# stdstu12/YUME

Measured on AMD Instinct MI355X. Metric: denoise-steps/sec (Yume-5B 720P, 33-frame latent), higher is better.
Workload: dtype bf16; 1 GPU; Yume-5B-720P random-init, 33-frame 704x1280 clip (latent 48x13x44x80, FramePack lfz=8, L=9460), ODE Euler steps of a 50-step shift-7 schedule, no CFG, one chain per GPU; num_layers=30, parallelism=dp1 (independent chains, replicated weights)

## Files before the change

include/yume_hip.h:

```cpp
#ifndef YUME_HIP_H
#define YUME_HIP_H

#include <stdint.h>

#ifdef __cplusplus
extern "C" {
#endif

#define YUME_OK 0
#define YUME_EINVAL (-1)
#define YUME_ELAUNCH (-2)
#define YUME_EUNSUP (-3)

const char* yume_last_error(void);
#define YUME_ABI_VERSION 9
int yume_abi_version(void);
const char* yume_target_arch(void);

int64_t yume_counter_workspace_bytes(void);
int yume_counter_workspace_init(void* ptr, int64_t bytes, void* stream);

int yume_calibrate_mfma(int64_t iters, int64_t workgroups, void* ticks, void* sink, void* stream);

int yume_adaln_modulate(const float* x, int64_t ldx, int64_t T, int64_t C, float eps,
                        const float* mul, const float* add, int64_t tab_stride,
                        const int32_t* row_idx, int add_one,
                        void* out, int64_t ldo, int out_kind, void* stream);

enum {
    YUME_EPI_BF16 = 0,
    YUME_EPI_BF16_GELU = 1,
    YUME_EPI_F32 = 2,
    YUME_EPI_RESID = 3,
    YUME_EPI_BF16_SPLITT = 4,
    YUME_EPI_BF16_GELU_ERF = 5,
    YUME_EPI_BF16_GEGLU = 6,
    YUME_EPI_MX_GELU = 7,
    YUME_EPI_MX6_GELU = 8
};
int yume_gemm_bf16(const void* A, int64_t lda, const void* W, int64_t ldw, const float* bias,
                   int64_t M, int64_t N, int64_t K, int epi,
                   void* out, int64_t ldo,
                   const float* gate, int64_t gate_stride, const int32_t* row_idx,
                   void* outT, int64_t ldt, int64_t n_split,
                   int variant, void* stream);

int64_t yume_gemm_workspace_bytes(void);
int yume_gemm_bf16_ws(const void* A, int64_t lda, const void* W, int64_t ldw, const float* bias,
                      int64_t M, int64_t N, int64_t K, int epi,
                      void* out, int64_t ldo,
                      const float* gate, int64_t gate_stride, const int32_t* row_idx,
                      void* outT, int64_t ldt, int64_t n_split,
                      int variant, void* workspace, int64_t workspace_bytes, void* stream);

int yume_quant_rows_e4m3(const void* x, int64_t ldx, int64_t R, int64_t K, void* q, int64_t ldq, float* scale, void* stream);
int yume_gemm_f8(const void* Aq, int64_t lda, const float* sa, const void* Wq, int64_t ldw, const float* sw,
                 const float* bias, int64_t M, int64_t N, int64_t K, int epi, void* out, int64_t ldo,
                 const float* gate, int64_t gate_stride, const int32_t* row_idx, void* stream);
int yume_gemm_f8_splitt(const void* Aq, int64_t lda, const float* sa, const void* Wq, int64_t ldw, const float* sw,
                        const float* bias, int64_t M, int64_t N, int64_t K,
                        void* out, int64_t ldo, void* outT, int64_t ldt, int64_t n_split, void* stream);

int yume_adaln_modulate_e4m3(const float* x, int64_t ldx, int64_t T, int64_t C, float eps, const float* mul,
                             const float* add, int64_t tab_stride, const int32_t* row_idx, int add_one,
                             void* q, int64_t ldq, float* scale, void* stream);
int yume_gemm_f8_mxout(const void* Aq, int64_t lda, const float* sa, const void* Wq, int64_t ldw, const float* sw,
                       const float* bias, int64_t M, int64_t N, int64_t K, int epi, void* out, int64_t ldo,
                       void* eo, int64_t ldeo, void* stream);
int yume_gemm_f8_mx(const void* Aq, int64_t lda, const void* ea, int64_t ldea, const void* Wq, int64_t ldw, const float* sw,
                    const float* bias, int64_t M, int64_t N, int64_t K, int epi, void* out, int64_t ldo,
                    const float* gate, int64_t gate_stride, const int32_t* row_idx, void* stream);

int yume_adaln_modulate_mx_e2m3(const float* x, int64_t ldx, int64_t T, int64_t C, float eps, const float* mul,
                                const float* add, int64_t tab_stride, const int32_t* row_idx, int add_one,
                                void* q, int64_t ldq, void* e, int64_t lde, void* stream);
int yume_gemm_f6_mx(const void* A6, int64_t lda, const void* ea, int64_t ldea, const void* W6, int64_t ldw, const void* ew, int64_t ldew,
                    const float* bias, int64_t M, int64_t N, int64_t K, int epi, void* out, int64_t ldo,
                    const float* gate, int64_t gate_stride, const int32_t* row_idx, void* stream);
int yume_gemm_f6_mxout(const void* A6, int64_t lda, const void* ea, int64_t ldea, const void* W6, int64_t ldw, const void* ew, int64_t ldew,
                       const float* bias, int64_t M, int64_t N, int64_t K, int epi, void* out, int64_t ldo,
                       void* eo, int64_t ldeo, void* stream);

int yume_quant_rows_i8(const void* x, int64_t ldx, int64_t R, int64_t K, void* q, int64_t ldq, float* scale, void* stream);
int yume_adaln_modulate_i8(const float* x, int64_t ldx, int64_t T, int64_t C, float eps, const float* mul,
                           const float* add, int64_t tab_stride, const int32_t* row_idx, int add_one,
                           void* q, int64_t ldq, float* scale, void* stream);
int yume_gemm_i8(const void* Aq, int64_t lda, const float* sa, const void* Wq, int64_t ldw, const float* sw,
                 const float* bias, int64_t M, int64_t N, int64_t K, int epi, void* out, int64_t ldo, void* stream);
int yume_gemm_i8_splitt(const void* Aq, int64_t lda, const float* sa, const void* Wq, int64_t ldw, const float* sw,
                        const float* bias, int64_t M, int64_t N, int64_t K,
                        void* out, int64_t ldo, void* outT, int64_t ldt, int64_t n_split, void* stream);

int yume_rmsnorm_rope(void* buf, int64_t ld, int64_t T, int64_t C, int nparts,
                      const float* w, float eps, const float* rope, int64_t D, void* stream);
int yume_rmsnorm_rows_periodic(void* buf, int64_t ld, int64_t T, int64_t C, const float* w, int64_t wperiod, float eps,
                               void* stream);

#define YUME_ATTN_Q_PRESCALED 0x100
#define YUME_ATTN_KV_PADDED 0x200
int yume_attn_fwd(const void* Q, int64_t ldq, const void* K, int64_t ldk, const void* Vt, int64_t ldvt,
                  void* O, int64_t ldo, int64_t Lq, int64_t Lk, int64_t H, float scale,
                  int accumulate, int variant, void* stream);
int64_t yume_attn_workspace_bytes(int64_t Lq, int64_t Lk, int64_t H);
int yume_attn_fwd_ws(const void* Q, int64_t ldq, const void* K, int64_t ldk, const void* Vt, int64_t ldvt,
                     void* O, int64_t ldo, int64_t Lq, int64_t Lk, int64_t H, float scale,
                     int accumulate, int variant, void* workspace, int64_t workspace_bytes, void* stream);
int yume_attn_fwd_kw(const void* Q, int64_t ldq, const void* K, int64_t ldk, const void* Vt, int64_t ldvt,
                     void* O, int64_t ldo, int64_t Lq, int64_t Lk, int64_t H, float scale,
                     int accumulate, int variant, void* workspace, int64_t workspace_bytes, float last_key_weight, void* stream);
int yume_attn_fwd_band(const void* Q, int64_t ldq, const void* K, int64_t ldk, const void* Vt, int64_t ldvt,
                       void* O, int64_t ldo, int64_t Lq, int64_t Lk, int64_t H, float scale, int accumulate, int variant,
                       int64_t q_pos0, int64_t win_left, int64_t win_right,
                       void* workspace, int64_t workspace_bytes, void* stream);
int yume_attn_fwd_seg(const void* Q, int64_t ldq, const void* const* K, int64_t ldk, const void* const* Vt, int64_t ldvt,
                      void* O, int64_t ldo, int64_t nseg, int64_t Lq_seg, int64_t seg_pitch, const int64_t* Lk, int64_t H,
                      float scale, int accumulate, int variant, const float* last_key_weight, void* stream);
int64_t yume_attn_batch_workspace_bytes(int64_t nseg, int64_t Lq_seg, int64_t Lk_seg, int64_t H);
int yume_attn_fwd_batch(const void* Q, int64_t ldq, const void* K, int64_t ldk, const void* Vt, int64_t ldvt,
                        void* O, int64_t ldo, int64_t nseg, int64_t Lq_seg, int64_t q_pitch,
                        int64_t Lk_seg, int64_t k_pitch, int64_t H, float scale, int accumulate, int variant,
                        void* workspace, int64_t workspace_bytes, void* stream);

int yume_quant_rows_mx_e4m3(const void* x, int64_t ldx, int64_t R, int64_t K, void* q, int64_t ldq, void* e, int64_t lde, void* stream);
int yume_attn_vt_mx_e4m3(const void* Vt, int64_t ldvt, int64_t C, int64_t Lk, void* Vt8, int64_t ldvt8, void* Ev, int64_t ldev, void* stream);
int yume_attn_fwd_f8mx(const void* Q8, int64_t ldq, const void* Eq, int64_t ldeq, const void* K8, int64_t ldk, const void* Ek, int64_t ldek,
                       const void* Vt8, int64_t ldvt8, const void* Ev, int64_t ldev, void* O, int64_t ldo,
                       int64_t Lq, int64_t Lk, int64_t H, void* stream);

int yume_linear_smallm_f32(const float* in, int64_t R, int64_t K, const void* W, int w_bf16,
                           const float* bias, int64_t N, int in_act, int out_act,
                           const float* add_table, float* out, void* stream);

int yume_sinusoidal_embed(const double* t, const int32_t* t_index, int64_t R, int64_t dim,
                          float* out, void* stream);

int yume_modulation_table(const float* tab, const float* e0, int64_t B, int64_t R, int64_t W,
// ... 69 lines not shown
```

yume_amd/_lib.py:

```python
import ctypes
import os
from ctypes import c_void_p, c_int, c_int64, c_float, c_char_p

_HERE = os.path.dirname(os.path.abspath(__file__))
LIB_PATH = os.environ.get("YUME_HIP_LIB") or os.path.join(_HERE, "lib", "libyume_hip.so")

_P, _I, _L, _F = c_void_p, c_int, c_int64, c_float

SIGNATURES = {
    "yume_last_error": [],
    "yume_abi_version": [],
    "yume_target_arch": [],
    "yume_counter_workspace_bytes": [],
    "yume_counter_workspace_init": [_P, _L, _P],
    "yume_calibrate_mfma": [_L, _L, _P, _P, _P],
    "yume_adaln_modulate": [_P, _L, _L, _L, _F, _P, _P, _L, _P, _I, _P, _L, _I, _P],
    "yume_adaln_modulate_e4m3": [_P, _L, _L, _L, _F, _P, _P, _L, _P, _I, _P, _L, _P, _P],
    "yume_gemm_bf16": [_P, _L, _P, _L, _P, _L, _L, _L, _I, _P, _L, _P, _L, _P, _P, _L, _L, _I, _P],
    "yume_gemm_workspace_bytes": [],
    "yume_gemm_bf16_ws": [_P, _L, _P, _L, _P, _L, _L, _L, _I, _P, _L, _P, _L, _P, _P, _L, _L, _I, _P, _L, _P],
    "yume_quant_rows_e4m3": [_P, _L, _L, _L, _P, _L, _P, _P],
    "yume_gemm_f8": [_P, _L, _P, _P, _L, _P, _P, _L, _L, _L, _I, _P, _L, _P, _L, _P, _P],
    "yume_gemm_f8_splitt": [_P, _L, _P, _P, _L, _P, _P, _L, _L, _L, _P, _L, _P, _L, _L, _P],
    "yume_gemm_f8_mxout": [_P, _L, _P, _P, _L, _P, _P, _L, _L, _L, _I, _P, _L, _P, _L, _P],
    "yume_gemm_f8_mx": [_P, _L, _P, _L, _P, _L, _P, _P, _L, _L, _L, _I, _P, _L, _P, _L, _P, _P],
    "yume_adaln_modulate_mx_e2m3": [_P, _L, _L, _L, _F, _P, _P, _L, _P, _I, _P, _L, _P, _L, _P],
    "yume_gemm_f6_mx": [_P, _L, _P, _L, _P, _L, _P, _L, _P, _L, _L, _L, _I, _P, _L, _P, _L, _P, _P],
    "yume_gemm_f6_mxout": [_P, _L, _P, _L, _P, _L, _P, _L, _P, _L, _L, _L, _I, _P, _L, _P, _L, _P],
    "yume_quant_rows_i8": [_P, _L, _L, _L, _P, _L, _P, _P],
    "yume_adaln_modulate_i8": [_P, _L, _L, _L, _F, _P, _P, _L, _P, _I, _P, _L, _P, _P],
    "yume_gemm_i8": [_P, _L, _P, _P, _L, _P, _P, _L, _L, _L, _I, _P, _L, _P],
    "yume_gemm_i8_splitt": [_P, _L, _P, _P, _L, _P, _P, _L, _L, _L, _P, _L, _P, _L, _L, _P],
    "yume_rmsnorm_f32": [_P, _L, _L, _L, _F, _P, _P, _L, _P],
    "yume_gemm_bf16_batched": [_P, _L, _L, _P, _L, _L, _L, _L, _L, _I, _P, _L, _L, _L, _I, _P],
    "yume_gemm_splitk_workspace_bytes": [_L, _L, _I],
    "yume_gemm_bf16_splitk": [_P, _L, _P, _L, _P, _L, _L, _L, _I, _P, _L, _I, _P, _P],
    "yume_softmax_bias_rows": [_P, _L, _L, _L, _L, _P, _L, _P, _L, _L, _P],
    "yume_rmsnorm_rows_periodic": [_P, _L, _L, _L, _P, _L, _F, _P],
    "yume_rmsnorm_rope": [_P, _L, _L, _L, _I, _P, _F, _P, _L, _P],
    "yume_attn_fwd": [_P, _L, _P, _L, _P, _L, _P, _L, _L, _L, _L, _F, _I, _I, _P],
    "yume_attn_workspace_bytes": [_L, _L, _L],
    "yume_attn_fwd_ws": [_P, _L, _P, _L, _P, _L, _P, _L, _L, _L, _L, _F, _I, _I, _P, _L, _P],
    "yume_attn_fwd_kw": [_P, _L, _P, _L, _P, _L, _P, _L, _L, _L, _L, _F, _I, _I, _P, _L, _F, _P],
    "yume_attn_fwd_band": [_P, _L, _P, _L, _P, _L, _P, _L, _L, _L, _L, _F, _I, _I, _L, _L, _L, _P, _L, _P],
    "yume_attn_fwd_seg": [_P, _L, _P, _L, _P, _L, _P, _L, _L, _L, _L, _P, _L, _F, _I, _I, _P, _P],
    "yume_attn_batch_workspace_bytes": [_L, _L, _L, _L],
    "yume_attn_fwd_batch": [_P, _L, _P, _L, _P, _L, _P, _L, _L, _L, _L, _L, _L, _L, _F, _I, _I, _P, _L, _P],
    "yume_quant_rows_mx_e4m3": [_P, _L, _L, _L, _P, _L, _P, _L, _P],
    "yume_attn_vt_mx_e4m3": [_P, _L, _L, _L, _P, _L, _P, _L, _P],
    "yume_attn_fwd_f8mx": [_P, _L, _P, _L, _P, _L, _P, _L, _P, _L, _P, _L, _P, _L, _L, _L, _L, _P],
    "yume_linear_smallm_f32": [_P, _L, _L, _P, _I, _P, _L, _I, _I, _P, _P, _P],
    "yume_sinusoidal_embed": [_P, _P, _L, _L, _P, _P],
    "yume_modulation_table": [_P, _P, _L, _L, _L, _P, _P],
    "yume_patch_gather": [_P, _I, _L, _L, _L, _L, _L, _L, _L, _L, _P, _L, _P],
    "yume_unpatchify": [_P, _L, _L, _L, _L, _L, _L, _L, _P, _P],
    "yume_cast_bf16": [_P, _L, _L, _L, _L, _P, _L, _P],
    "yume_transpose_bf16": [_P, _I, _L, _L, _L, _P, _L, _P],
    "yume_conv3d_cl": [_P, _P, _L, _L, _L, _L, _L, _P, _L, _P, _L, _I, _I, _I, _I, _I, _I, _I, _I, _I, _I, _L, _L, _L, _I, _P, _L,
                       _P, _L, _P, _P],
    "yume_vae_rmsnorm_silu": [_P, _L, _L, _L, _P, _P, _I, _P, _L, _P],
    "yume_vae_rmsnorm_silu_mx": [_P, _L, _L, _L, _P, _P, _I, _P, _L, _P, _L, _P],
    "yume_conv3d_cl_f8mx": [_P, _P, _P, _P, _L, _L, _L, _L, _L, _L, _P, _L, _P, _P, _L, _I, _I, _I, _I, _I, _I, _I, _I, _I, _I, _L, _L, _L,
                            _I, _P, _L, _P, _L, _P, _P],
    "yume_conv_up2_fold": [_P, _L, _L, _L, _L, _L, _P, _L, _P, _L, _P, _L, _P],
    "yume_vae_dupup_add": [_P, _L, _L, _L, _L, _L, _P, _L, _L, _L, _I, _I, _I, _P],
    "yume_vae_avgdown_add": [_P, _L, _L, _L, _L, _L, _P, _L, _L, _I, _I, _P],
    "yume_softmax_rows": [_P, _L, _L, _L, _F, _P, _L, _P],
    "yume_vae_pack_input": [_P, _I, _L, _L, _L, _L, _I, _P, _P, _P, _L, _P],
    "yume_frames_u8": [_P, _L, _L, _L, _L, _P, _P],
    "yume_frames_u8_trunc": [_P, _L, _L, _L, _L, _P, _P],
    "yume_vae_unpack_output": [_P, _L, _L, _L, _L, _L, _I, _P, _P, _F, _F, _P, _P],
}
_RES = {"yume_last_error": c_char_p, "yume_target_arch": c_char_p, "yume_gemm_splitk_workspace_bytes": c_int64, "yume_attn_workspace_bytes": c_int64,
        "yume_attn_batch_workspace_bytes": c_int64,
        "yume_counter_workspace_bytes": c_int64, "yume_gemm_workspace_bytes": c_int64}

_lib = None
ABI_VERSION = 9


def load():
    global _lib
    if _lib is not None:
        return _lib
    if not os.path.exists(LIB_PATH):
        raise RuntimeError(
            f"{LIB_PATH} is missing: the HIP extension has not been built. "
            "Run `python -c 'import __graft_entry__ as g; g.build()'` (or `python -m yume_amd.build`). "
            "There is no CPU/PyTorch fallback for the yume_amd hot path.")
    import torch
    lib = ctypes.CDLL(LIB_PATH)
    for name, argtypes in SIGNATURES.items():
        fn = getattr(lib, name)
        fn.argtypes = argtypes
        fn.restype = _RES.get(name, c_int)
    got, arch = int(lib.yume_abi_version()), lib.yume_target_arch()
    if got != ABI_VERSION or arch != b"gfx950":
        raise RuntimeError(f"{LIB_PATH} has ABI version {got} for {arch!r}, this binding needs {ABI_VERSION} for gfx950: "
                           "rebuild with `python -m yume_amd.build --force`")
    _lib = lib
    return lib


def check(rc, what):
    if rc != 0:
        msg = load().yume_last_error()
        raise RuntimeError(f"{what} failed (rc={rc}): {msg.decode() if msg else '?'}")
```

yume_amd/csrc/gemm_bf16.hip:

```cpp
#include "gemm_core.hpp"
#include "gemm_w4.hpp"

using namespace gemm_core;

namespace {
bool w4_auto() {
    static const bool on = [] { const char* v = getenv("YUME_GEMM_W4"); return !v || atoi(v) != 0; }();
    return on;
}
bool gemm_log() {
    static const bool on = [] { const char* v = getenv("YUME_GEMM_LOG"); return v && atoi(v) != 0; }();
    return on;
}
void gemm_log_line(const char* kernel, int64_t M, int64_t N, int64_t K, int epi, int variant, int64_t lda, int64_t ldw, int64_t ldo, int64_t ldt,
                   int64_t n_split, bool ws, int64_t batch) {
    fprintf(stderr, "[gemm_bf16] %s M=%lld N=%lld K=%lld epi=%d variant=%d lda=%lld ldw=%lld ldo=%lld ldt=%lld n_split=%lld ws=%d batch=%lld\n", kernel,
            (long long)M, (long long)N, (long long)K, epi, variant, (long long)lda, (long long)ldw, (long long)ldo, (long long)ldt, (long long)n_split,
            ws ? 1 : 0, (long long)batch);
}
}

extern "C" int64_t yume_gemm_workspace_bytes(void) { return gemm_w4::sk_workspace_bytes(gemm_w4::SK_MAX_SLOTS); }

extern "C" int yume_gemm_bf16(const void* A, int64_t lda, const void* W, int64_t ldw, const float* bias, int64_t M,
                              int64_t N, int64_t K, int epi, void* out, int64_t ldo, const float* gate,
                              int64_t gate_stride, const int32_t* row_idx, void* outT, int64_t ldt, int64_t n_split,
                              int variant, void* stream) {
    return yume_gemm_bf16_ws(A, lda, W, ldw, bias, M, N, K, epi, out, ldo, gate, gate_stride, row_idx, outT, ldt, n_split, variant, nullptr, 0, stream);
}

extern "C" int yume_gemm_bf16_ws(const void* A, int64_t lda, const void* W, int64_t ldw, const float* bias, int64_t M,
                                 int64_t N, int64_t K, int epi, void* out, int64_t ldo, const float* gate,
                                 int64_t gate_stride, const int32_t* row_idx, void* outT, int64_t ldt, int64_t n_split,
                                 int variant, void* workspace, int64_t workspace_bytes, void* stream) {
    YUME_REQUIRE(A && W && out, "gemm_bf16: NULL pointer");
    YUME_REQUIRE(M > 0 && N > 0 && K > 0, "gemm_bf16: empty problem M=%lld N=%lld K=%lld", (long long)M, (long long)N, (long long)K);
    YUME_REQUIRE(M < (1ll << 31) && N < (1ll << 31) && K < (1ll << 31), "gemm_bf16: dimension too large");
    YUME_REQUIRE((K % BK) == 0, "gemm_bf16: K=%lld must be a multiple of %d", (long long)K, BK);
    YUME_REQUIRE((N % 4) == 0, "gemm_bf16: N=%lld must be a multiple of 4", (long long)N);
    YUME_REQUIRE((lda % 8) == 0 && (ldw % 8) == 0, "gemm_bf16: lda/ldw must be multiples of 8 (16-byte rows)");
    YUME_REQUIRE((ldo % 4) == 0, "gemm_bf16: ldo must be a multiple of 4");
    YUME_REQUIRE(((uintptr_t)A % 16) == 0 && ((uintptr_t)W % 16) == 0 && ((uintptr_t)out % 16) == 0, "gemm_bf16: pointers must be 16-byte aligned");
    Problem p;
    p.W = (const unsigned short*)W; p.ldw = ldw;
    p.M = (int)M; p.N = (int)N; p.K = (int)K;
    p.tiles_m = (int)((M + BM - 1) / BM);
    p.tiles_n = (int)((N + BN - 1) / BN);
    p.group_m = 8;
    p.bsW = 0; p.bsO = 0;
    bool sk = false;
    if (variant == 0 && workspace != nullptr && w4_auto() && epi != YUME_EPI_BF16_GEGLU &&
        use_256(p, 0, epi != YUME_EPI_BF16_SPLITT || (n_split % 256) == 0) && gemm_w4::w4_applies(p, lda, epi) &&
        (epi != YUME_EPI_BF16_SPLITT || (ldt % 8) == 0)) {
        Problem q = p;
        q.tiles_m = (int)((M + 255) / 256);
        q.tiles_n = (int)((N + 255) / 256);
        gemm_w4::w4_sk_plan(q, workspace, workspace_bytes);
        sk = q.sk_wgs != 0;
    }
    if (!sk && variant == 0 && epi != YUME_EPI_BF16_GEGLU && use_256(p, 0, epi != YUME_EPI_BF16_SPLITT || (n_split % 256) == 0)) {
        const int64_t tn = (N + 255) / 256, tm = (M + 255) / 256, T = tm * tn, R = T % 256, full = T - R;
        const int64_t m_main = full / tn, M_main = m_main * 256, rem = M - M_main;
        if (R > 0 && R <= 96 && full >= 256 && m_main >= 1 && rem > 0 && rem <= 1024) {
            const int64_t osz = (epi == YUME_EPI_F32 || epi == YUME_EPI_RESID) ? 4 : 2;
            auto remainder = [&](void* s2) {
                return yume_gemm_bf16(reinterpret_cast<const unsigned short*>(A) + M_main * lda, lda, W, ldw, bias, rem, N, K, epi,
                                      reinterpret_cast<char*>(out) + M_main * ldo * osz, ldo, gate, gate_stride,
                                      row_idx ? row_idx + M_main : nullptr,
                                      outT ? reinterpret_cast<unsigned short*>(outT) + M_main : nullptr, ldt, n_split, 1, s2);
            };
            int rc = yume_gemm_bf16(A, lda, W, ldw, bias, M_main, N, K, epi, out, ldo, gate, gate_stride, row_idx, outT, ldt, n_split,
                                    w4_auto() ? 3 : 2, stream);
            if (rc != YUME_OK) return rc;
            return remainder(stream);
        }
    }
    PlainA al;
    al.A = (const unsigned short*)A; al.lda = lda; al.M = (int)M; al.bsA = 0;
    Epilogue e = {};
    e.bias = bias;
    e.out = out; e.ldo = ldo;
    e.gate = gate; e.gate_stride = gate_stride; e.row_idx = row_idx;
    e.outT = (unsigned short*)outT; e.ldt = ldt; e.n_split = (int)n_split;
    hipStream_t st = (hipStream_t)stream;
    const bool split_ok = epi != YUME_EPI_BF16_SPLITT || (n_split % 256) == 0;
    const bool big = use_256(p, variant == 3 ? 2 : variant, split_ok);
    const bool w4 = (variant == 3 || (variant == 0 && big && w4_auto())) && split_ok && gemm_w4::w4_applies(p, lda, epi) &&
                    (epi != YUME_EPI_BF16_SPLITT || (ldt % 8) == 0);
    if (gemm_log())
        gemm_log_line(epi == YUME_EPI_BF16_GEGLU ? "g256" : w4 ? (sk ? "w4+sk" : "w4") : big ? "g256" : "g128", M, N, K, epi, variant, lda, ldw, ldo, ldt,
                      n_split, workspace != nullptr, 1);
#define YUME_GO(E) (w4 ? gemm_w4::launch_w4(E, p, al, e, st, "gemm_bf16", variant == 0 ? workspace : nullptr, workspace_bytes) : big ? launch256<E>(p, al, e, st, "gemm_bf16") : launch<E>(p, al, e, st, "gemm_bf16"))
    switch (epi) {
        case YUME_EPI_BF16: return YUME_GO(YUME_EPI_BF16);
        case YUME_EPI_BF16_GELU: return YUME_GO(YUME_EPI_BF16_GELU);
        case YUME_EPI_BF16_GELU_ERF: return YUME_GO(YUME_EPI_BF16_GELU_ERF);
        case YUME_EPI_F32: return YUME_GO(YUME_EPI_F32);
        case YUME_EPI_RESID:
            YUME_REQUIRE(gate == nullptr || (gate_stride % 4) == 0, "gemm_bf16: gate_stride must be a multiple of 4");
            return YUME_GO(YUME_EPI_RESID);
        case YUME_EPI_BF16_GEGLU:
            YUME_REQUIRE((N % 8) == 0 && bias == nullptr, "gemm_bf16: GEGLU needs N %% 8 == 0 and no bias");
            return launch256<YUME_EPI_BF16_GEGLU>(p, al, e, st, "gemm_bf16");
        case YUME_EPI_BF16_SPLITT:
            YUME_REQUIRE(outT != nullptr && n_split >= 0 && (n_split % BN) == 0 && ldt >= M && (ldt % 4) == 0,
                         "gemm_bf16: SPLITT needs outT, n_split %% 128 == 0, ldt >= M and ldt %% 4 == 0");
            YUME_REQUIRE(((uintptr_t)outT % 16) == 0, "gemm_bf16: outT must be 16-byte aligned");
            return YUME_GO(YUME_EPI_BF16_SPLITT);
        default:
            yume_set_error("gemm_bf16: unknown epilogue %d", epi);
            return YUME_EINVAL;
    }
}

extern "C" int yume_gemm_bf16_batched(const void* A, int64_t lda, int64_t strideA, const void* W, int64_t ldw, int64_t strideW,
                                      int64_t M, int64_t N, int64_t K, int epi, void* out, int64_t ldo, int64_t strideO,
                                      int64_t batch, int variant, void* stream) {
    (void)variant;
    YUME_REQUIRE(A && W && out, "gemm_bf16_batched: NULL pointer");
    YUME_REQUIRE(epi == YUME_EPI_BF16 || epi == YUME_EPI_F32, "gemm_bf16_batched: only the plain bf16 / fp32 epilogues");
    YUME_REQUIRE(batch >= 1 && batch <= 65535, "gemm_bf16_batched: batch %lld", (long long)batch);
    YUME_REQUIRE(M > 0 && N > 0 && K > 0 && M < (1ll << 31) && N < (1ll << 31) && K < (1ll << 31), "gemm_bf16_batched: bad problem size");
    YUME_REQUIRE((K % BK) == 0 && (N % 4) == 0, "gemm_bf16_batched: K must be a multiple of %d and N of 4", BK);
    YUME_REQUIRE((lda % 8) == 0 && (ldw % 8) == 0 && (ldo % 4) == 0, "gemm_bf16_batched: lda/ldw must be multiples of 8, ldo of 4");
    YUME_REQUIRE((strideA % 8) == 0 && (strideW % 8) == 0 && (strideO % 8) == 0, "gemm_bf16_batched: strides must keep 16-byte alignment");
    YUME_REQUIRE(((uintptr_t)A % 16) == 0 && ((uintptr_t)W % 16) == 0 && ((uintptr_t)out % 16) == 0, "gemm_bf16_batched: pointers must be 16-byte aligned");
    Problem p;
    p.W = (const unsigned short*)W; p.ldw = ldw;
    p.M = (int)M; p.N = (int)N; p.K = (int)K;
    p.tiles_m = (int)((M + BM - 1) / BM);
    p.tiles_n = (int)((N + BN - 1) / BN);
    p.group_m = 8;
    p.bsW = strideW;
    p.bsO = strideO * (epi == YUME_EPI_F32 ? 4 : 2);
    PlainA al;
    al.A = (const unsigned short*)A; al.lda = lda; al.M = (int)M; al.bsA = strideA;
    Epilogue e = {};
    e.out = out; e.ldo = ldo;
    hipStream_t st = (hipStream_t)stream;
    if (gemm_log()) gemm_log_line("batched", M, N, K, epi, variant, lda, ldw, ldo, 0, 0, false, batch);
    if (epi == YUME_EPI_F32) return launch<YUME_EPI_F32>(p, al, e, st, "gemm_bf16_batched", (int)batch);
    return launch<YUME_EPI_BF16>(p, al, e, st, "gemm_bf16_batched", (int)batch);
}

namespace {
template <int EPI>
__global__ __launch_bounds__(256) void splitk_reduce_kernel(const float* __restrict__ ws, int splits, int64_t MN, int N,
                                                            const float* __restrict__ bias, void* __restrict__ out, int64_t ldo) {
    const int64_t nq = MN >> 2;
    for (int64_t i = (int64_t)blockIdx.x * blockDim.x + threadIdx.x; i < nq; i += (int64_t)gridDim.x * blockDim.x) {
        f32x4 v = *reinterpret_cast<const f32x4*>(ws + 4 * i);
        for (int s = 1; s < splits; ++s) v += *reinterpret_cast<const f32x4*>(ws + s * MN + 4 * i);
        const int64_t m = (4 * i) / N;
        const int n = (int)((4 * i) - m * N);
        if (bias) v += *reinterpret_cast<const f32x4*>(bias + n);
        if (EPI == YUME_EPI_F32) {
            *reinterpret_cast<f32x4*>(reinterpret_cast<float*>(out) + m * ldo + n) = v;
        } else if (EPI == YUME_EPI_RESID) {
            float* xo = reinterpret_cast<float*>(out) + m * ldo + n;
            *reinterpret_cast<f32x4*>(xo) = *reinterpret_cast<const f32x4*>(xo) + v;
        } else if (EPI == YUME_EPI_BF16_GEGLU) {
            const unsigned o = pack_bf16x2(v[1] * gelu_tanh(v[0]), v[3] * gelu_tanh(v[2]));
            *reinterpret_cast<unsigned*>(reinterpret_cast<unsigned short*>(out) + m * ldo + (n >> 1)) = o;
        } else {
            if (EPI == YUME_EPI_BF16_GELU) {
#pragma unroll
                for (int q = 0; q < 4; ++q) v[q] = gelu_tanh(v[q]);
            }
            if (EPI == YUME_EPI_BF16_GELU_ERF) {
#pragma unroll
                for (int q = 0; q < 4; ++q) v[q] = 0.5f * v[q] * (1.0f + erff(v[q] * 0.7071067811865476f));
            }
            u32x2 o;
            o[0] = pack_bf16x2(v[0], v[1]);
            o[1] = pack_bf16x2(v[2], v[3]);
            *reinterpret_cast<u32x2*>(reinterpret_cast<unsigned short*>(out) + m * ldo + n) = o;
        }
    }
}
}

extern "C" int64_t yume_gemm_splitk_workspace_bytes(int64_t M, int64_t N, int splits) { return (int64_t)splits * M * N * 4; }

extern "C" int yume_gemm_bf16_splitk(const void* A, int64_t lda, const void* W, int64_t ldw, const float* bias, int64_t M, int64_t N,
                                     int64_t K, int epi, void* out, int64_t ldo, int splits, void* workspace, void* stream) {
    YUME_REQUIRE(A && W && out && workspace, "gemm_bf16_splitk: NULL pointer");
    YUME_REQUIRE(splits >= 1 && splits <= 64 && (K % (splits * BK)) == 0, "gemm_bf16_splitk: K=%lld must be a multiple of splits*%d (splits=%d)",
                 (long long)K, BK, splits);
    YUME_REQUIRE(M > 0 && N > 0 && (N % 8) == 0 && (ldo % 4) == 0, "gemm_bf16_splitk: N must be a multiple of 8, ldo of 4");
    YUME_REQUIRE(((uintptr_t)workspace % 16) == 0 && ((uintptr_t)out % 16) == 0, "gemm_bf16_splitk: pointers must be 16-byte aligned");
    YUME_REQUIRE((M * N) % 4 == 0, "gemm_bf16_splitk: M*N must be a multiple of 4");
    const int64_t Ks = K / splits;
    int rc = yume_gemm_bf16_batched(A, lda, Ks, W, ldw, Ks, M, N, Ks, YUME_EPI_F32, workspace, N, M * N, splits, 1, stream);
    if (rc != YUME_OK) return rc;
    const int64_t MN = M * N;
    const unsigned grid = (unsigned)((MN / 4 + 255) / 256 > 16384 ? 16384 : (MN / 4 + 255) / 256);
    hipStream_t st = (hipStream_t)stream;
// ... 20 lines not shown
```

yume_amd/csrc/gemm_w4.hpp:

```cpp
#pragma once
#include "gemm_core.hpp"
#include "trace.hpp"

namespace gemm_w4 {
using namespace gemm_core;

constexpr int NTHR_W4 = 256;
constexpr int OPER_BYTES = 256 * 128;
constexpr int BUF_BYTES = 2 * OPER_BYTES;
constexpr int LDS_W4 = 2 * BUF_BYTES;

#define W4_AG8(n) "a" #n "0", "a" #n "1", "a" #n "2", "a" #n "3", "a" #n "4", "a" #n "5", "a" #n "6", "a" #n "7", "a" #n "8", "a" #n "9"
#define W4_AGPRS "a0", "a1", "a2", "a3", "a4", "a5", "a6", "a7", "a8", "a9", W4_AG8(1), W4_AG8(2), W4_AG8(3), W4_AG8(4), W4_AG8(5), W4_AG8(6), \
    W4_AG8(7), W4_AG8(8), W4_AG8(9), W4_AG8(10), W4_AG8(11), W4_AG8(12), W4_AG8(13), W4_AG8(14), W4_AG8(15), W4_AG8(16), W4_AG8(17), W4_AG8(18), \
    W4_AG8(19), W4_AG8(20), W4_AG8(21), W4_AG8(22), W4_AG8(23), W4_AG8(24), "a250", "a251", "a252", "a253", "a254", "a255"

#define W4_MFMA2(T0, X0, Y0, T1, X1, Y1)                                                                                                         \
    asm volatile("v_mfma_f32_16x16x32_bf16 a[%c4:%c5], %0, %1, a[%c4:%c5]\n\tv_mfma_f32_16x16x32_bf16 a[%c6:%c7], %2, %3, a[%c6:%c7]"             \
                 ::"v"(X0), "v"(Y0), "v"(X1), "v"(Y1), "n"((T0) * 4), "n"((T0) * 4 + 3), "n"((T1) * 4), "n"((T1) * 4 + 3) : "memory", W4_AGPRS)
#define W4_MFMA2_DMA(T0, X0, Y0, T1, X1, Y1, voff, sbase, lbase, loff)                                                                            \
    asm volatile("s_add_u32 m0, %10, %11\n\tv_mfma_f32_16x16x32_bf16 a[%c4:%c5], %0, %1, a[%c4:%c5]\n\tglobal_load_lds_dwordx4 %8, %9\n\t"         \
                 "v_mfma_f32_16x16x32_bf16 a[%c6:%c7], %2, %3, a[%c6:%c7]"                                                                       \
                 ::"v"(X0), "v"(Y0), "v"(X1), "v"(Y1), "n"((T0) * 4), "n"((T0) * 4 + 3), "n"((T1) * 4), "n"((T1) * 4 + 3), "v"(voff), "s"(sbase),   \
                 "s"(lbase), "n"(loff) : "memory", "scc", W4_AGPRS)
// ... 550 lines not shown
            tails = true;
            const int ntail = (p.sk_s - 1) * R;
            pc0 = (w - R) * p.sk_q;
            pc1 = min(ntail, pc0 + p.sk_q);
            if (pc0 >= pc1) return;
        }
    }
    for (int pc = pc0; pc < pc1; ++pc) {
        int t = head_t, j = 0, k0 = 0, k1 = nk, slot = -1, nslice = 1;
        if (p.sk_wgs && (int)blockIdx.x >= ndp) {
            if (tails) {
                j = 1 + pc / R;
                t = pc - (j - 1) * R;
                k0 = p.sk_lh + (j - 1) * p.sk_lt;
                k1 = j == p.sk_s - 1 ? nk : k0 + p.sk_lt;
                slot = pc;
            } else {
                k1 = p.sk_lh;
                nslice = p.sk_s;
            }
        }
        int m0, n0;
        tile_origin(p, tile0 + t, m0, n0);
        if (epi == YUME_EPI_BF16_SPLITT && n0 >= e.n_split) {
            w4_mainloop<false>(p, al, smem, m0, n0, k0, k1 - k0);
            w4_finish_piece<false>(p, e, epi, smem, m0, n0, slot, t, nslice);
        } else {
            w4_mainloop<true>(p, al, smem, m0, n0, k0, k1 - k0);
            w4_finish_piece<true>(p, e, epi, smem, m0, n0, slot, t, nslice);
        }
        if (pc + 1 < pc1) __syncthreads();
    }
    TRACE_STAMP(2);
}

inline bool w4_applies(const Problem& p, int64_t lda, int epi) {
    if (p.K < 3 * BK) return false;
#ifdef W4_EXPERIMENT
    if (epi != YUME_EPI_BF16) return false;
#endif
    if (255ll * lda * 2 + 128 >= (1ll << 32) || 255ll * p.ldw * 2 + 128 >= (1ll << 32)) return false;
    return epi == YUME_EPI_BF16 || epi == YUME_EPI_BF16_GELU || epi == YUME_EPI_BF16_GELU_ERF || epi == YUME_EPI_F32 || epi == YUME_EPI_RESID ||
           epi == YUME_EPI_BF16_SPLITT;
}

inline void w4_sk_plan(Problem& p, void* ws, int64_t ws_bytes) {
    p.sk_dp = 0; p.sk_tiles = 0; p.sk_wgs = 0; p.sk_s = 1; p.sk_q = 1; p.sk_lh = 0; p.sk_lt = 0; p.sk_ws = nullptr;
    static const bool on = [] { const char* v = getenv("YUME_GEMM_SK"); return !v || atoi(v) != 0; }();
    static const int ncu = [] {
        int d = 0, n = 0;
        if (hipGetDevice(&d) != hipSuccess || hipDeviceGetAttribute(&n, hipDeviceAttributeMultiprocessorCount, d) != hipSuccess) n = 0;
        return n;
    }();
    if (!on || ws == nullptr || ncu < 64 || ncu > SK_MAX_SLOTS || (ncu & 7) != 0) return;
    if (ws_bytes < sk_workspace_bytes(SK_MAX_SLOTS) || ((uintptr_t)ws & 15) != 0) return;
    const int T = p.tiles_m * p.tiles_n, nk = p.K / BK;
    const int R = T % ncu;
    if (R == 0 || T < ncu) return;
    static const int min_nk = [] { const char* v = getenv("YUME_GEMM_SK_MIN_NK"); return v ? atoi(v) : 96; }();
    if (nk < min_nk) return;
    int s, q, lh, lt;
    if (2 * R > ncu) {
        s = 2;
        q = (R + (ncu - R) - 1) / (ncu - R);
        lt = nk / (q + 1);
        lh = nk - lt;
    } else {
        s = ncu / R;
        if (s > nk / SK_MIN_KT) s = nk / SK_MIN_KT;
        q = 1;
        lt = nk / s;
        lh = lt;
    }
    if (s < 2 || lt < SK_MIN_KT || lh < SK_MIN_KT || (s - 1) * R > SK_MAX_SLOTS) return;
    const int nwg = R + ((s - 1) * R + q - 1) / q;
    if (nwg > ncu) return;
    p.sk_tiles = R;
    p.sk_dp = T - R;
    p.sk_s = s; p.sk_q = q; p.sk_lh = lh; p.sk_lt = lt;
    p.sk_wgs = (nwg + 7) / 8 * 8;
    p.sk_ws = (char*)ws;
}

inline int launch_w4(int epi, const Problem& p128, const PlainA& al, const Epilogue& e, hipStream_t st, const char* what, void* ws = nullptr,
                     int64_t ws_bytes = 0) {
    Problem p = p128;
    p.tiles_m = (p.M + 255) / 256;
    p.tiles_n = (p.N + 255) / 256;
    p.group_m = g_group_m;
    { static const int d = [] { const char* v = getenv("YUME_GEMM_EPI_DIRECT"); return v ? atoi(v) : 0; }(); p.epi_direct = d; }
    w4_sk_plan(p, ws, ws_bytes);
    const unsigned grid = p.sk_wgs ? (unsigned)(p.sk_dp + p.sk_wgs) : (unsigned)(p.tiles_m * p.tiles_n);
    hipLaunchKernelGGL(gemm_w4_kernel<0>, dim3(grid), dim3(NTHR_W4), 0, st, p, al, e, epi);
    YUME_CHECK_LAUNCH(what);
    return YUME_OK;
}

}
```

Baseline: 10.33 denoise-steps/sec.

## Split bf16 GEMMs into a 256x256 front band and a 256x192 tail kernel

Adds a second bf16 GEMM kernel with 256x192 tiles and a planner that splits M. The first rows run on the existing 256x256 kernel in whole waves of CUs, and the remaining rows run on the narrower-tile kernel. The aim is to cut wave-quantization waste on the last partial wave of tiles for bf16 and residual epilogues. It adds a second launch per GEMM and a hand-scheduled mainloop whose cost model uses a fixed 0.78 tile-cost constant. It is enabled by default through YUME_GEMM_BAND.

```diff
diff --git a/include/yume_hip.h b/include/yume_hip.h
--- a/include/yume_hip.h
+++ b/include/yume_hip.h
@@ -52,6 +52,13 @@
                       const float* gate, int64_t gate_stride, const int32_t* row_idx,
                       void* outT, int64_t ldt, int64_t n_split,
                       int variant, void* workspace, int64_t workspace_bytes, void* stream);
+
+int64_t yume_gemm_band_plan(int64_t M, int64_t N, int ncu);
+int yume_gemm_bf16_band(const void* A, int64_t lda, const void* W, int64_t ldw, const float* bias,
+                        int64_t M, int64_t N, int64_t K, int epi,
+                        void* out, int64_t ldo,
+                        const float* gate, int64_t gate_stride, const int32_t* row_idx,
+                        int64_t band_m0, void* stream);
 
 int yume_quant_rows_e4m3(const void* x, int64_t ldx, int64_t R, int64_t K, void* q, int64_t ldq, float* scale, void* stream);
 int yume_gemm_f8(const void* Aq, int64_t lda, const float* sa, const void* Wq, int64_t ldw, const float* sw,
diff --git a/yume_amd/_lib.py b/yume_amd/_lib.py
--- a/yume_amd/_lib.py
+++ b/yume_amd/_lib.py
@@ -19,6 +19,8 @@
     "yume_gemm_bf16": [_P, _L, _P, _L, _P, _L, _L, _L, _I, _P, _L, _P, _L, _P, _P, _L, _L, _I, _P],
     "yume_gemm_workspace_bytes": [],
     "yume_gemm_bf16_ws": [_P, _L, _P, _L, _P, _L, _L, _L, _I, _P, _L, _P, _L, _P, _P, _L, _L, _I, _P, _L, _P],
+    "yume_gemm_band_plan": [_L, _L, _I],
+    "yume_gemm_bf16_band": [_P, _L, _P, _L, _P, _L, _L, _L, _I, _P, _L, _P, _L, _P, _L, _P],
     "yume_quant_rows_e4m3": [_P, _L, _L, _L, _P, _L, _P, _P],
     "yume_gemm_f8": [_P, _L, _P, _P, _L, _P, _P, _L, _L, _L, _I, _P, _L, _P, _L, _P, _P],
     "yume_gemm_f8_splitt": [_P, _L, _P, _P, _L, _P, _P, _L, _L, _L, _P, _L, _P, _L, _L, _P],
@@ -73,7 +75,7 @@
 }
 _RES = {"yume_last_error": c_char_p, "yume_target_arch": c_char_p, "yume_gemm_splitk_workspace_bytes": c_int64, "yume_attn_workspace_bytes": c_int64,
         "yume_attn_batch_workspace_bytes": c_int64,
-        "yume_counter_workspace_bytes": c_int64, "yume_gemm_workspace_bytes": c_int64}
+        "yume_counter_workspace_bytes": c_int64, "yume_gemm_workspace_bytes": c_int64, "yume_gemm_band_plan": c_int64}
 
 _lib = None
 ABI_VERSION = 9
diff --git a/yume_amd/csrc/gemm_bf16.hip b/yume_amd/csrc/gemm_bf16.hip
--- a/yume_amd/csrc/gemm_bf16.hip
+++ b/yume_amd/csrc/gemm_bf16.hip
@@ -1,5 +1,6 @@
 #include "gemm_core.hpp"
 #include "gemm_w4.hpp"
+#include "gemm_w4b.hpp"
 
 using namespace gemm_core;
 
@@ -11,6 +12,18 @@
 bool gemm_log() {
     static const bool on = [] { const char* v = getenv("YUME_GEMM_LOG"); return v && atoi(v) != 0; }();
     return on;
+}
+bool band_auto() {
+    static const bool on = [] { const char* v = getenv("YUME_GEMM_BAND"); return !v || atoi(v) != 0; }();
+    return on;
+}
+int device_cus() {
+    static const int ncu = [] {
+        int d = 0, n = 0;
+        if (hipGetDevice(&d) != hipSuccess || hipDeviceGetAttribute(&n, hipDeviceAttributeMultiprocessorCount, d) != hipSuccess) n = 0;
+        return n;
+    }();
+    return ncu;
 }
 void gemm_log_line(const char* kernel, int64_t M, int64_t N, int64_t K, int epi, int variant, int64_t lda, int64_t ldw, int64_t ldo, int64_t ldt,
                    int64_t n_split, bool ws, int64_t batch) {
@@ -74,6 +87,12 @@
             if (rc != YUME_OK) return rc;
             return remainder(stream);
         }
+    }
+    if (!sk && variant == 0 && band_auto() && w4_auto() && (epi == YUME_EPI_BF16 || epi == YUME_EPI_RESID) && use_256(p, 0, true) &&
+        gemm_w4::w4_applies(p, lda, epi) && gemm_w4b::w4b_applies(p, lda, epi)) {
+        const int64_t band_m0 = gemm_w4b::band_plan(M, N, device_cus());
+        if (band_m0 > 0)
+            return yume_gemm_bf16_band(A, lda, W, ldw, bias, M, N, K, epi, out, ldo, gate, gate_stride, row_idx, band_m0, stream);
     }
     PlainA al;
     al.A = (const unsigned short*)A; al.lda = lda; al.M = (int)M; al.bsA = 0;
@@ -113,6 +132,42 @@
     }
 }
 
+extern "C" int64_t yume_gemm_band_plan(int64_t M, int64_t N, int ncu) { return gemm_w4b::band_plan(M, N, ncu); }
+
+extern "C" int yume_gemm_bf16_band(const void* A, int64_t lda, const void* W, int64_t ldw, const float* bias, int64_t M, int64_t N, int64_t K,
+                                   int epi, void* out, int64_t ldo, const float* gate, int64_t gate_stride, const int32_t* row_idx,
+                                   int64_t band_m0, void* stream) {
+    YUME_REQUIRE(A && W && out, "gemm_bf16_band: NULL pointer");
+    YUME_REQUIRE(M > 0 && N > 0 && K > 0, "gemm_bf16_band: empty problem M=%lld N=%lld K=%lld", (long long)M, (long long)N, (long long)K);
+    YUME_REQUIRE(M < (1ll << 31) && N < (1ll << 31) && K < (1ll << 31), "gemm_bf16_band: dimension too large");
+    YUME_REQUIRE((K % BK) == 0 && K >= 3 * BK, "gemm_bf16_band: K=%lld must be a multiple of %d and at least %d", (long long)K, BK, 3 * BK);
+    YUME_REQUIRE((N % gemm_w4b::BN_B) == 0, "gemm_bf16_band: N=%lld must be a multiple of %d", (long long)N, gemm_w4b::BN_B);
+    YUME_REQUIRE(epi == YUME_EPI_BF16 || epi == YUME_EPI_RESID, "gemm_bf16_band: only the bf16 and residual epilogues (epi=%d)", epi);
+    YUME_REQUIRE(band_m0 >= 0 && band_m0 < M && (band_m0 % 256) == 0, "gemm_bf16_band: band_m0=%lld must be a multiple of 256 inside M=%lld",
+                 (long long)band_m0, (long long)M);
+    YUME_REQUIRE((lda % 8) == 0 && (ldw % 8) == 0, "gemm_bf16_band: lda/ldw must be multiples of 8 (16-byte rows)");
+    YUME_REQUIRE((ldo % 4) == 0, "gemm_bf16_band: ldo must be a multiple of 4");
+    YUME_REQUIRE(((uintptr_t)A % 16) == 0 && ((uintptr_t)W % 16) == 0 && ((uintptr_t)out % 16) == 0, "gemm_bf16_band: pointers must be 16-byte aligned");
+    YUME_REQUIRE(epi != YUME_EPI_RESID || gate == nullptr || (gate_stride % 4) == 0, "gemm_bf16_band: gate_stride must be a multiple of 4");
+    if (band_m0 > 0) {
+        const int rc = yume_gemm_bf16(A, lda, W, ldw, bias, band_m0, N, K, epi, out, ldo, gate, gate_stride, row_idx, nullptr, 0, 0, 3, stream);
+        if (rc != YUME_OK) return rc;
+    }
+    const int64_t rows = M - band_m0, osz = epi == YUME_EPI_RESID ? 4 : 2;
+    Problem p = {};
+    p.W = (const unsigned short*)W; p.ldw = ldw;
+    p.M = (int)rows; p.N = (int)N; p.K = (int)K;
+    PlainA al;
+    al.A = (const unsigned short*)A + band_m0 * lda; al.lda = lda; al.M = (int)rows; al.bsA = 0;
+    YUME_REQUIRE(gemm_w4b::w4b_applies(p, lda, epi), "gemm_bf16_band: row strides beyond the kernel's 32-bit source offsets");
+    Epilogue e = {};
+    e.bias = bias;
+    e.out = reinterpret_cast<char*>(out) + band_m0 * ldo * osz; e.ldo = ldo;
+    e.gate = gate; e.gate_stride = gate_stride; e.row_idx = row_idx ? row_idx + band_m0 : nullptr;
+    if (gemm_log()) gemm_log_line("w4b", rows, N, K, epi, 0, lda, ldw, ldo, 0, 0, false, 1);
+    return gemm_w4b::launch_w4b(epi, p, al, e, (hipStream_t)stream, "gemm_bf16_band");
+}
+
 extern "C" int yume_gemm_bf16_batched(const void* A, int64_t lda, int64_t strideA, const void* W, int64_t ldw, int64_t strideW,
                                       int64_t M, int64_t N, int64_t K, int epi, void* out, int64_t ldo, int64_t strideO,
                                       int64_t batch, int variant, void* stream) {
diff --git a/yume_amd/csrc/gemm_w4.hpp b/yume_amd/csrc/gemm_w4.hpp
--- a/yume_amd/csrc/gemm_w4.hpp
+++ b/yume_amd/csrc/gemm_w4.hpp
@@ -656,6 +656,7 @@
     p.sk_ws = (char*)ws;
 }
 
+#ifndef W4_NO_LAUNCHER
 inline int launch_w4(int epi, const Problem& p128, const PlainA& al, const Epilogue& e, hipStream_t st, const char* what, void* ws = nullptr,
                      int64_t ws_bytes = 0) {
     Problem p = p128;
@@ -669,5 +670,6 @@
     YUME_CHECK_LAUNCH(what);
     return YUME_OK;
 }
-
-}
+#endif
+
+}
diff --git a/yume_amd/csrc/gemm_w4b.hip b/yume_amd/csrc/gemm_w4b.hip
--- /dev/null
+++ b/yume_amd/csrc/gemm_w4b.hip
@@ -0,0 +1,313 @@
+#define W4_NO_LAUNCHER
+#include "gemm_w4.hpp"
+#include "gemm_w4b.hpp"
+
+namespace gemm_w4b {
+using namespace gemm_core;
+using gemm_w4::acc_tile;
+using gemm_w4::acc_zero;
+using gemm_w4::static_for;
+
+constexpr int NTHR_B = 256;
+constexpr int A_BYTES = 256 * 128;
+constexpr int W_BYTES = BN_B * 128;
+constexpr int BUF_STRIDE = 65536;
+constexpr int LDS_B = BUF_STRIDE + A_BYTES + W_BYTES;
+constexpr int NPIECE = 14;
+constexpr int NSLOT = 48;
+
+struct CtxB {
+    char* smem;
+    bf16x8_t fa[2][8], fb[2][6];
+    unsigned ra1, rb1, ra0n, rb0n;
+    unsigned va[8], vb[6];
+    const char* pa;
+    const char* pb;
+    unsigned lcur;
+};
+
+__device__ __forceinline__ bf16x8_t frag(const CtxB& c, unsigned off) { return *reinterpret_cast<const bf16x8_t*>(c.smem + off); }
+
+#define W4B_X(g) c.fb[(g) / 48][((g) % 48) % 6]
+#define W4B_Y(g) c.fa[(g) / 48][((g) % 48) / 6]
+#define W4B_PAIR(g) W4_MFMA2((g) % 48, W4B_X(g), W4B_Y(g), ((g) + 1) % 48, W4B_X((g) + 1), W4B_Y((g) + 1))
+#define W4B_PAIR_DMA(g, voff, sbase, loff) \
+    W4_MFMA2_DMA((g) % 48, W4B_X(g), W4B_Y(g), ((g) + 1) % 48, W4B_X((g) + 1), W4B_Y((g) + 1), voff, sbase, c.lcur, loff)
+
+constexpr int PB_BAR_A = 14;
+constexpr int PB_BAR_B = 26;
+constexpr int PB_DMA0 = PB_BAR_A + 2;
+constexpr int PB_F0_FIRST = PB_BAR_B + 2;
+constexpr int dma_pos(int q) { return PB_DMA0 + (q * (NSLOT - 1 - PB_DMA0)) / (NPIECE - 1); }
+constexpr int piece_at(int pos) {
+    for (int q = 0; q < NPIECE; ++q)
+        if (dma_pos(q) == pos) return q;
+    return -1;
+}
+constexpr int pieces_before_bar_b() {
+    int k = 0;
+    for (int q = 0; q < NPIECE; ++q) k += dma_pos(q) <= PB_BAR_B ? 1 : 0;
+    return k;
+}
+constexpr bool dma_pos_distinct() {
+    for (int q = 1; q < NPIECE; ++q)
+        if (dma_pos(q) <= dma_pos(q - 1)) return false;
+    return true;
+}
+static_assert(NPIECE - 1 < PB_BAR_A && dma_pos(0) > PB_BAR_A && dma_pos(NPIECE - 1) <= NSLOT - 1 && dma_pos_distinct() && PB_BAR_B >= NSLOT / 2 &&
+                  PB_F0_FIRST + NPIECE <= NSLOT,
+              "the plan must fit the 48 slots");
+
+template <int g, bool DMA>
+__device__ __forceinline__ void gaps(CtxB& c) {
+    if constexpr (g < 2 * NSLOT) {
+        constexpr int pos = g >> 1;
+        constexpr int q = DMA ? piece_at(pos) : -1;
+        if constexpr (q >= 0 && q < 8) W4B_PAIR_DMA(g, c.va[q & 7], c.pa, q * 4096);
+        else if constexpr (q >= 8) W4B_PAIR_DMA(g, c.vb[q >= 8 ? q - 8 : 0], c.pb, q * 4096);
+        else W4B_PAIR(g);
+        if constexpr (pos < NPIECE) {
+            if constexpr (pos < 6) c.fb[1][pos % 6] = frag(c, c.rb1 + (pos % 6) * 2048);
+            else c.fa[1][(pos - 6) & 7] = frag(c, c.ra1 + ((pos - 6) & 7) * 2048);
+        }
+        if constexpr (pos == PB_BAR_A) asm volatile("s_waitcnt lgkmcnt(0)\n\ts_barrier" ::: "memory");
+        if constexpr (pos == PB_BAR_B) {
+            constexpr int keep = DMA ? pieces_before_bar_b() : 0;
+            asm volatile("s_waitcnt vmcnt(%c0)\n\ts_barrier" ::"n"(keep) : "memory");
+        }
+        if constexpr (pos >= PB_F0_FIRST && pos < PB_F0_FIRST + NPIECE) {
+            constexpr int r = pos - PB_F0_FIRST;
+            if constexpr (r < 6) c.fb[0][r % 6] = frag(c, c.rb0n + (r % 6) * 2048);
+            else c.fa[0][(r - 6) & 7] = frag(c, c.ra0n + ((r - 6) & 7) * 2048);
+        }
+        gaps<g + 2, DMA>(c);
+    }
+}
+template <int q>
+__device__ __forceinline__ void stage_all(CtxB& c) {
+    if constexpr (q < NPIECE) {
+        if constexpr (q < 8) W4_DMA(c.va[q & 7], c.pa, c.lcur, q * 4096);
+        else W4_DMA(c.vb[q >= 8 ? q - 8 : 0], c.pb, c.lcur, q * 4096);
+        stage_all<q + 1>(c);
+    }
+}
+
+template <bool DMA>
+__device__ __forceinline__ void loop(CtxB& c, int t0, int t1, unsigned lbase) {
+    for (int t = t0; t < t1; ++t) {
+        gaps<0, DMA>(c);
+        if constexpr (DMA) {
+            c.pa += 128;
+            c.pb += 128;
+        }
+        c.lcur = lbase + (((t + 1) & 1) ? BUF_STRIDE : 0);
+        c.ra1 ^= BUF_STRIDE;
+        c.rb1 ^= BUF_STRIDE;
+        c.ra0n ^= BUF_STRIDE;
+        c.rb0n ^= BUF_STRIDE;
+    }
+}
+
+__device__ __forceinline__ void mainloop(const Problem& p, const PlainA& al, char* smem, int m0, int n0, int nk) {
+    const int tid = threadIdx.x;
+    const int lane = tid & 63;
+    const int wave = __builtin_amdgcn_readfirstlane(tid >> 6);
+    const int wr = wave >> 1, wc = wave & 1;
+    CtxB c;
+    c.smem = smem;
+    const unsigned lbase = (unsigned)(uintptr_t)(__attribute__((address_space(3))) char*)smem + wave * 1024;
+    c.lcur = lbase;
+    c.pa = reinterpret_cast<const char*>(al.A + (int64_t)m0 * al.lda);
+    c.pb = reinterpret_cast<const char*>(p.W + (int64_t)n0 * p.ldw);
+    const unsigned lda_b = (unsigned)al.lda * 2u, ldw_b = (unsigned)p.ldw * 2u;
+    {
+        const int rl = 8 * wave + (lane >> 3);
+        const unsigned ch = (unsigned)(((lane & 7) ^ (rl & 7)) << 4);
+        const int mleft = p.M - 1 - m0, nleft = p.N - 1 - n0;
+#pragma unroll
+        for (int j = 0; j < 8; ++j) c.va[j] = (unsigned)min(32 * j + rl, mleft) * lda_b + ch;
+#pragma unroll
+        for (int j = 0; j < 6; ++j) c.vb[j] = (unsigned)min(32 * j + rl, nleft) * ldw_b + ch;
+    }
+    const unsigned sw0 = (unsigned)(((lane >> 4) ^ (lane & 7)) << 4), sw1 = (unsigned)(((4 | (lane >> 4)) ^ (lane & 7)) << 4);
+    const unsigned rowa = wr * 16384 + (lane & 15) * 128, rowb = A_BYTES + wc * (96 * 128) + (lane & 15) * 128;
+    stage_all<0>(c);
+    c.pa += 128;
+    c.pb += 128;
+    c.lcur = lbase + BUF_STRIDE;
+    stage_all<0>(c);
+    c.pa += 128;
+    c.pb += 128;
+    c.lcur = lbase;
+    acc_zero<0, 192>();
+    asm volatile("s_waitcnt vmcnt(%c0)\n\ts_barrier" ::"n"(NPIECE) : "memory");
+#pragma unroll
+    for (int r = 0; r < 6; ++r) c.fb[0][r] = frag(c, rowb + sw0 + r * 2048);
+#pragma unroll
+    for (int r = 0; r < 8; ++r) c.fa[0][r] = frag(c, rowa + sw0 + r * 2048);
+    c.ra1 = rowa + sw1;
+    c.rb1 = rowb + sw1;
+    c.ra0n = BUF_STRIDE + rowa + sw0;
+    c.rb0n = BUF_STRIDE + rowb + sw0;
+    loop<true>(c, 0, nk - 2, lbase);
+    loop<false>(c, nk - 2, nk, lbase);
+    asm volatile("s_waitcnt lgkmcnt(0)\n\ts_barrier" ::: "memory");
+    asm volatile("s_nop 15\n\ts_nop 15" ::: "memory");
+}
+
+__device__ __forceinline__ void store_image(char* smem, unsigned short* dst, int64_t ld, int row0, int rows_valid, int col0) {
+    const int lane = threadIdx.x & 63;
+    const int wave = __builtin_amdgcn_readfirstlane(threadIdx.x >> 6);
+    const int rh = lane >= 48 ? 2 : lane >= 24 ? 1 : 0, cl = lane - 24 * rh;
+    if (rh == 2) return;
+    const int rleft = rows_valid - wave * 64 - rh;
+    char* o = reinterpret_cast<char*>(dst + col0 + cl * 8) + (int64_t)(row0 + wave * 64 + rh) * ld * 2;
+    const int64_t step = ld * 4;
+#pragma unroll
+    for (int g = 0; g < 4; ++g) {
+        u32x4 d[8];
+#pragma unroll
+        for (int u = 0; u < 8; ++u) {
+            const int it = g * 8 + u;
+            const int r = wave * 64 + 2 * it + rh;
+            d[u] = *reinterpret_cast<const u32x4*>(smem + r * 384 + ((cl ^ (r & 7)) << 4));
+        }
+#pragma unroll
+        for (int u = 0; u < 8; ++u) {
+            const int it = g * 8 + u;
+            if (2 * it < rleft) *reinterpret_cast<u32x4*>(o + it * step) = d[u];
+        }
+    }
+}
+
+template <int EPI>
+__device__ __forceinline__ void epilogue(const Problem& p, const Epilogue& e, int m0, int n0, char* smem) {
+    const int lane = threadIdx.x & 63;
+    const int wave = __builtin_amdgcn_readfirstlane(threadIdx.x >> 6);
+    const int wr = wave >> 1, wc = wave & 1;
+    const int l15 = lane & 15, l4 = lane >> 4;
+    if (EPI == YUME_EPI_BF16 && !p.epi_direct && (e.ldo % 8) == 0) {
+        f32x4 b[6];
+#pragma unroll
+        for (int j = 0; j < 6; ++j) b[j] = e.bias ? *reinterpret_cast<const f32x4*>(e.bias + n0 + wc * 96 + 16 * j + 4 * l4) : f32x4{0.f, 0.f, 0.f, 0.f};
+        unsigned io[6];
+#pragma unroll
+        for (int j = 0; j < 6; ++j)
+            io[j] = (unsigned)((wr * 128 + l15) * 384 + (((12 * wc + 2 * j + (l4 >> 1)) ^ (l15 & 7)) << 4) + (l4 & 1) * 8);
+        static_for<0, 8>([&](auto ii) {
+            constexpr int i = decltype(ii)::value;
+            static_for<0, 6>([&](auto jj) {
+                constexpr int j = decltype(jj)::value;
+                const f32x4 v = acc_tile<i * 6 + j>() + b[j];
+                u32x2 o;
+                o[0] = pack_bf16x2(v[0], v[1]);
+                o[1] = pack_bf16x2(v[2], v[3]);
+                *reinterpret_cast<u32x2*>(smem + io[j] + i * (16 * 384)) = o;
+            });
+        });
+        asm volatile("s_waitcnt lgkmcnt(0)\n\ts_barrier" ::: "memory");
+        store_image(smem, reinterpret_cast<unsigned short*>(e.out), e.ldo, m0, min(256, p.M - m0), n0);
+        return;
+    }
+    if (EPI == YUME_EPI_RESID) {
+        f32x4 b[6];
+#pragma unroll
+        for (int j = 0; j < 6; ++j) b[j] = e.bias ? *reinterpret_cast<const f32x4*>(e.bias + n0 + wc * 96 + 16 * j + 4 * l4) : f32x4{0.f, 0.f, 0.f, 0.f};
+        const int mrow = m0 + wr * 128 + l15, ncol = n0 + wc * 96 + 4 * l4;
+        const bool ragged_m = m0 + 256 > p.M;
+        const int mlast = p.M - 1 - mrow;
+        float* const xo = reinterpret_cast<float*>(e.out) + (int64_t)mrow * e.ldo + ncol;
+        const int64_t xstep = 16 * e.ldo;
+        auto xoff = [&](int i) -> int64_t { return ragged_m ? (int64_t)(min(16 * i, mlast)) * e.ldo : i * xstep; };
+        const bool gated = e.gate != nullptr;
+        bool rowed = gated && e.row_idx != nullptr;
+        int ridx[8];
+#pragma unroll
+        for (int i = 0; i < 8; ++i) ridx[i] = rowed ? e.row_idx[min(mrow + 16 * i, p.M - 1)] : 0;
+        f32x4 x[2][6], g[2][6];
+        auto issue_x = [&](auto ii, auto bb) {
+            constexpr int i = decltype(ii)::value, bf = decltype(bb)::value;
+#pragma unroll
+            for (int j = 0; j < 6; ++j) x[bf][j] = *reinterpret_cast<const f32x4*>(xo + xoff(i) + 16 * j);
+        };
+        auto issue_g = [&](auto ii, auto bb) {
+            constexpr int i = decltype(ii)::value, bf = decltype(bb)::value;
+            if (rowed || (gated && i < 2)) {
+                const float* gp = e.gate + (int64_t)ridx[i] * e.gate_stride + ncol;
+#pragma unroll
+                for (int j = 0; j < 6; ++j) g[bf][j] = *reinterpret_cast<const f32x4*>(gp + 16 * j);
+            }
+        };
+        issue_x(std::integral_constant<int, 0>{}, std::integral_constant<int, 0>{});
+        issue_x(std::integral_constant<int, 1>{}, std::integral_constant<int, 1>{});
+        if (rowed) {
+            const int r0 = __builtin_amdgcn_readfirstlane(ridx[0]);
+            bool same = true;
+#pragma unroll
+            for (int i = 0; i < 8; ++i) same &= ridx[i] == r0;
+            if (__all(same)) rowed = false;
+        }
+        issue_g(std::integral_constant<int, 0>{}, std::integral_constant<int, 0>{});
+        issue_g(std::integral_constant<int, 1>{}, std::integral_constant<int, 1>{});
+        static_for<0, 8>([&](auto ii) {
+            constexpr int i = decltype(ii)::value, bf = i & 1;
+            static_for<0, 6>([&](auto jj) {
+                constexpr int j = decltype(jj)::value;
+                const f32x4 v = acc_tile<i * 6 + j>() + b[j];
+                if (gated) x[bf][j] += v * g[bf][j];
+                else x[bf][j] += v;
+                if (!ragged_m || 16 * i <= mlast) *reinterpret_cast<f32x4*>(xo + i * xstep + 16 * j) = x[bf][j];
+            });
+            if constexpr (i + 2 < 8) {
+                issue_x(std::integral_constant<int, i + 2>{}, std::integral_constant<int, bf>{});
+                issue_g(std::integral_constant<int, i + 2>{}, std::integral_constant<int, bf>{});
+            }
+        });
+        return;
+    }
+    static_for<0, 48>([&](auto tt) {
+        constexpr int T = decltype(tt)::value, i = T / 6, j = T % 6;
+        const f32x4 v = acc_tile<T>();
+        const int m = m0 + wr * 128 + 16 * i + l15, n = n0 + wc * 96 + 16 * j + 4 * l4;
+        if (m < p.M && n < p.N) store_row4<EPI>(v, m, n, p, e);
+    });
+}
+
+__device__ __forceinline__ void tile_origin_b(const Problem& p, int wg, int& m0, int& n0) {
+    const int width = p.group_m * p.tiles_n;
+    const int group = wg / width;
+    const int first_m = group * p.group_m;
+    const int gsz = min(p.tiles_m - first_m, p.group_m);
+    m0 = (first_m + (wg % width) % gsz) * 256;
+    n0 = ((wg % width) / gsz) * BN_B;
+}
+
+__global__ __launch_bounds__(NTHR_B, 1) void gemm_w4b_kernel(Problem p, PlainA al, Epilogue e, int epi) {
+    __shared__ __attribute__((aligned(16))) char smem[LDS_B];
+    int start, count, m0, n0;
+    xcd_chunk(p.tiles_m * p.tiles_n, blockIdx.x & 7, start, count);
+    tile_origin_b(p, start + (blockIdx.x >> 3), m0, n0);
+    mainloop(p, al, smem, m0, n0, p.K / BK);
+    if (epi == YUME_EPI_RESID) epilogue<YUME_EPI_RESID>(p, e, m0, n0, smem);
+    else epilogue<YUME_EPI_BF16>(p, e, m0, n0, smem);
+}
+
+bool w4b_applies(const Problem& p, int64_t lda, int epi) {
+    if (p.K < 3 * BK || (p.K % BK) != 0 || (p.N % BN_B) != 0) return false;
+    if (255ll * lda * 2 + 128 >= (1ll << 32) || 191ll * p.ldw * 2 + 128 >= (1ll << 32)) return false;
+    return epi == YUME_EPI_BF16 || epi == YUME_EPI_RESID;
+}
+
+int launch_w4b(int epi, const Problem& p0, const PlainA& al, const Epilogue& e, hipStream_t st, const char* what) {
+    Problem p = p0;
+    p.tiles_m = (p.M + 255) / 256;
+    p.tiles_n = p.N / BN_B;
+    p.group_m = g_group_m;
+    { static const int d = [] { const char* v = getenv("YUME_GEMM_EPI_DIRECT"); return v ? atoi(v) : 0; }(); p.epi_direct = d; }
+    p.sk_dp = 0; p.sk_tiles = 0; p.sk_wgs = 0; p.sk_s = 1; p.sk_q = 1; p.sk_lh = 0; p.sk_lt = 0; p.sk_ws = nullptr;
+    hipLaunchKernelGGL(gemm_w4b_kernel, dim3((unsigned)(p.tiles_m * p.tiles_n)), dim3(NTHR_B), 0, st, p, al, e, epi);
+    YUME_CHECK_LAUNCH(what);
+    return YUME_OK;
+}
+
+}
diff --git a/yume_amd/csrc/gemm_w4b.hpp b/yume_amd/csrc/gemm_w4b.hpp
--- /dev/null
+++ b/yume_amd/csrc/gemm_w4b.hpp
@@ -0,0 +1,31 @@
+#pragma once
+#include "gemm_core.hpp"
+
+namespace gemm_w4b {
+
+constexpr int BN_B = 192;
+constexpr double BAND_TILE_COST = 0.78;
+constexpr double BAND_MIN_GAIN = 0.08;
+
+inline int64_t band_plan(int64_t M, int64_t N, int ncu) {
+    if (M <= 0 || N <= 0 || ncu <= 0 || (N % BN_B) != 0 || (N % 256) != 0) return -1;
+    const int64_t tn = N / 256, tnb = N / BN_B, tm = (M + 255) / 256, T = tm * tn;
+    if (T < ncu) return -1;
+    const int64_t base = (T + ncu - 1) / ncu;
+    double best = 0.0;
+    int64_t best_b = -1;
+    for (int64_t r = 1; r <= base; ++r) {
+        const int64_t b = r * ncu / tn;
+        if (b < 1 || b >= tm) continue;
+        const int64_t front = (b * tn + ncu - 1) / ncu, band = ((tm - b) * tnb + ncu - 1) / ncu;
+        const double cost = (double)front + BAND_TILE_COST * (double)band;
+        if (best_b < 0 || cost < best) { best = cost; best_b = b; }
+    }
+    if (best_b < 0 || best > (1.0 - BAND_MIN_GAIN) * (double)base) return -1;
+    return best_b * 256;
+}
+
+bool w4b_applies(const gemm_core::Problem& p, int64_t lda, int epi);
+int launch_w4b(int epi, const gemm_core::Problem& p, const gemm_core::PlainA& al, const gemm_core::Epilogue& e, hipStream_t st, const char* what);
+
+}
```

Result: no change. 10.37 denoise-steps/sec, median of 6 (+0.3%).
